# Acelogic/Retrieval-based-Voice-Conversion-MLX

Measured on AMD Instinct MI355X. Metric: audio-sec/sec (realtime factor) RVCv2 48kHz pipeline, higher is better.
Workload: dtype fp32-accurate (two-plane fp16 MFMA split); 1 GPU; C2: full RVCv2 48kHz pipeline, one 13.5 s utterance per step per GPU; samples_16k=216100, x_pad=1, f0_method=rmvpe, parallelism=dp1

## Files before the change

### retrieval-based-voice-conversion-mlx_amd/csrc/conv2d_small.hip

```cpp
#include <hip/hip_runtime.h>

#include <cstdlib>

#include "split_bf16.h"

namespace rvcx {

namespace {
typedef float f32x4 __attribute__((ext_vector_type(4)));

}

constexpr int SIT = 17;

template <int CIN, int NOUT, int PIX>
__global__ __launch_bounds__(256) void k_conv2d_small(const ConvArgs a, const int RH) {
  constexpr int CP = CIN + 4;
  constexpr int NT = NOUT / 16;
  constexpr int CG = CIN / 16;
  constexpr int TPW = PIX / 64;
  extern __shared__ __attribute__((aligned(16))) float sm[];
  const int W = a.W_out, H = a.T_out;
  const int AW = W + 2;
  float* As = sm;
// ... 396 lines not shown
                   (a.res_mode == RES_NONE || a.res_mode == RES_ADD_POST) &&
                   (a.act == ACT_NONE || a.act == ACT_RELU || a.act == ACT_LRELU) && a.w_bs == 0 && a.bias_bs == 0;
  const bool align = (a.ldx % 4 == 0) && (a.x_bs % 4 == 0) && (a.ldw % 4 == 0) && (a.w_ts % 4 == 0) &&
                     ((reinterpret_cast<uintptr_t>(a.x) & 15) == 0) && ((reinterpret_cast<uintptr_t>(a.w) & 15) == 0) &&
                     a.ldx >= a.C_in && a.ldw >= a.C_in;
  return epi && align;
}

static int s2d_nt(const ConvArgs& a) { return a.N <= 16 ? 1 : 2; }
long long small2d_wsplit_bytes(const ConvArgs& a) {
  return (long long)(a.C_in == 16 ? 5 : 9) * s2d_nt(a) * 2 * 1024 + 256;
}
hipError_t small2d_wsplit_build(const ConvArgs& a, void* out, hipStream_t s) {
  if (!conv2d_small_fits(a)) return hipErrorInvalidValue;
  hipLaunchKernelGGL(k_s2d_wsplit, dim3(1), dim3(256), 0, s, a.w, a.w_ts, a.ldw, a.N, a.C_in, s2d_nt(a),
                     static_cast<unsigned short*>(out));
  return hipGetLastError();
}

hipError_t conv2d_small(const ConvArgs& a, hipStream_t s) {
  if (a.wsplit && a.wsplit_fmt == WSPLIT_S2D) {
    hipError_t e = hipErrorInvalidValue;
    if (a.C_in == 16) e = a.N <= 16 ? launch_h16<16, 16>(a, s) : launch_h16<16, 32>(a, s);
    else e = a.N <= 16 ? launch_h16<32, 16>(a, s) : launch_h16<32, 32>(a, s);
    if (e != hipErrorInvalidValue) return e;
  }
  if (a.C_in == 16 && a.N <= 16) return launch_small<16, 16, 512>(a, s);
  if (a.C_in == 16 && a.N == 32) return launch_small<16, 32, 512>(a, s);
  if (a.C_in == 32 && a.N <= 16) return launch_small<32, 16, 256>(a, s);
  if (a.C_in == 32 && a.N == 32) return launch_small<32, 32, 256>(a, s);
  return hipErrorInvalidValue;
}

}
```

### retrieval-based-voice-conversion-mlx_amd/csrc/conv_kernels.h

```cpp
#pragma once
#include "kernel_base.h"

namespace rvcx {

enum ResMode : int {
  RES_NONE = 0,
  RES_ADD_PRE = 1,
  RES_ADD_POST = 2,
  RES_RSUB_POST = 3,
};

enum AccMode : int {
  ACC_STORE = 0,
  ACC_ADD = 1,
  ACC_ADD_DIV = 2,
};

enum OutMap : int {
  OUT_ROWS = 0,
  OUT_UPSAMPLE2D = 1,
};

enum WsplitFmt : int { WSPLIT_BF16 = 0, WSPLIT_H16 = 1, WSPLIT_S2D = 2 };

// ... 62 lines not shown
  const float* nz_w = nullptr;
  const float* nz_b = nullptr;
  int lds_pad = 0;
  const int* h_in = nullptr;
};

enum ConvKind : int { CK_WSB16 = 0, CK_WSB, CK_GS, CK_GSW, CK_RBPAIR, CK_SMALL2D, CK_EMU, CK_GEMM, CK_TINY, CK_WST,
                      CK_OTHER, CK_COUNT };
const char* conv_kind_name(int k);
enum ConvTile : int {
  TILE_NONE = -1,
  TILE_F32_128x32 = 1, TILE_F32_64x64 = 3, TILE_EMU_128x32 = 12, TILE_EMU_64x64 = 13,
  TILE_WSB_128x64 = 23, TILE_WSB_256x32 = 24, TILE_WSB_128x128 = 25, TILE_WSB_128x64_1x4 = 27, TILE_GS_64x64 = 30,
};
struct ConvForce {
  int kind = -1, tile = TILE_NONE, pipe = 0;
};
struct ConvPlan {
  ConvKind kind;
  int tile, ksplit;
  long long slab_floats;
  int wsplit_fmt;
  bool needs_image, pipe;
};
ConvPlan conv_plan(const ConvArgs& a, bool two_d, bool static_weight, const ConvForce& force = ConvForce());
hipError_t conv_run(const ConvPlan& plan, const ConvArgs& a, bool two_d, hipStream_t s, bool forced = false);
int conv_math(int requested);


bool conv2d_small_fits(const ConvArgs& a);
hipError_t conv2d_small(const ConvArgs& a, hipStream_t s);
long long small2d_wsplit_bytes(const ConvArgs& a);
hipError_t small2d_wsplit_build(const ConvArgs& a, void* out, hipStream_t s);

bool conv_wsb_eligible(const ConvArgs& a, bool two_d = false);
bool conv_wsb_tile(int cfg, int& BM, int& BN);
int conv_wsplit_npad(int N);
long long conv_wsplit_bytes(const ConvArgs& a);
hipError_t conv_wsplit_build(const ConvArgs& a, void* out, hipStream_t s);
hipError_t conv_wsb_launch(const ConvArgs& a, int cfg, hipStream_t s, bool two_d = false,
                           int ksplit = 1);

bool conv_gs_eligible(const ConvArgs& a, bool two_d);
bool conv_gs_form(const ConvArgs& a, bool two_d);
bool conv_gsw_eligible(const ConvArgs& a);
hipError_t conv_gs_launch(const ConvArgs& a, int cfg, hipStream_t s, bool two_d, int ksplit);

bool conv_wst_fits(const ConvArgs& a, bool two_d);
hipError_t conv_wst_launch(const ConvArgs& a, hipStream_t s);

struct RbPairArgs {
  const float* x = nullptr;
  long long x_bs = 0;
  const void* w1s = nullptr;
  const float* b1 = nullptr;
  const void* w2s = nullptr;
  const float* b2 = nullptr;
  int C = 0, k = 0, d = 1, T = 0, B = 1;
  float* y = nullptr;
  long long y_bs = 0;
  int acc_mode = ACC_STORE;
  float acc_div = 1.f;
  int wfmt = 0;
  int lowp = 0;
};
enum RbWfmt : int { RB_WBF16 = 0, RB_WF16 = 1 };
// ... 7 lines not shown
```

### retrieval-based-voice-conversion-mlx_amd/csrc/runtime.h

```cpp
#pragma once
#include <hip/hip_runtime.h>

#include <cstdint>
#include <cstdlib>
#include <functional>
#include <map>
#include <memory>
#include <stdexcept>
#include <string>
#include <tuple>
#include <vector>

#include "../../include/rvcx.h"
#include "rvcx_kernels.h"

namespace rvcx {

struct Error : std::runtime_error {
  int code;
  Error(int c, const std::string& m) : std::runtime_error(m), code(c) {}
};

#define RVCX_HIP(expr)                                                                                 \
  do {                                                                                                 \
// ... 342 lines not shown
                         const float* rate, const float* one_minus_rate, float* out, hipStream_t s);
void index_reconstruct_n(Ctx& c, int64_t i0, int64_t ni, float* out, hipStream_t s);
void index_build(Ctx& c, const float* x, int64_t n, int d, int64_t nlist, const rvcx_index_build_opts& o,
                 hipStream_t s);
void index_centroids(Ctx& c, float* out, hipStream_t s);
int64_t index_save(Ctx& c, void* bytes, int64_t cap);
void kmeans_assign_run(Ctx& c, const float* x, int64_t n, int d, const float* cent, int64_t nlist, int32_t* assign,
                       float* dist, hipStream_t s);
void kmeans_update_run(Ctx& c, const float* x, int64_t n, int d, const int32_t* assign, int64_t nlist, float* cent,
                       int64_t* sizes, hipStream_t s);
int64_t pipeline_forward_ex(Ctx& c, const double* audio, int64_t n, const rvcx_pipeline_opts& o,
                            const float* eps_z, const float* eps_src, uint64_t seed, float* out, int64_t cap,
                            double* f0_out, hipStream_t s, bool sizing);
int64_t pipeline_forward_batch(Ctx& c, const double* audio, int64_t n, int64_t lda, int B, const rvcx_pipeline_opts& o,
                               const int32_t* sids, const float* eps_z, const float* eps_src, uint64_t seed,
                               float* out, int64_t ldo, double* f0_out, float* hidden_out, hipStream_t s);
void pipeline_forward_rows(Ctx& c, const double* audio, const int64_t* nv, int64_t lda, int B,
                           const rvcx_pipeline_opts& o, const int32_t* sids, const float* eps_z, const float* eps_src,
                           uint64_t seed, float* out, int64_t ldo, int64_t* n_out, double* f0_out, int64_t ldf,
                           float* hidden_out, hipStream_t s, bool sizing);
int64_t pipeline_workspace_bytes(Ctx& c, int B, int64_t n, const rvcx_pipeline_opts& o, hipStream_t s);
rvcx_pipeline_opts default_pipeline_opts();
int proposed_key(const std::vector<double>& f0, double threshold);
int64_t hubert_frames(int64_t n);
void set_i32(int32_t* p, int32_t v, hipStream_t s);
void set_i32_once(Ctx& c, const std::string& name, int32_t* p, int32_t v, hipStream_t s);
hipStream_t fork_aux(Ctx& c, hipStream_t s);
bool conv_routes_wsb16(Ctx& c, const ConvArgs& a);
void join_aux(Ctx& c, hipStream_t s, hipStream_t ax);
void launch_conv(Ctx& c, const ConvArgs& a_in, bool two_d, hipStream_t s, double flops = -1.0);
ConvPlan launch_conv_test(Ctx& c, const ConvArgs& a_in, bool two_d, bool static_weight, const ConvForce& force,
                          int expect_kind, const char* who, hipStream_t s);
void launch_rb_pair(Ctx& c, const RbPairArgs& a, hipStream_t s);
inline void check(hipError_t e, const char* what) {
  if (e != hipSuccess) throw Error(RVCX_E_HIP, std::string(what) + ": " + hipGetErrorString(e));
}

}
```

### retrieval-based-voice-conversion-mlx_amd/csrc/runtime_conv.cpp

```cpp
#include <algorithm>
#include <cstdlib>
#include <cstring>
#include <string>

#include "runtime.h"

namespace rvcx {
hipStream_t Ctx::aux_stream() {
  if (!aux) {
    RVCX_HIP(hipSetDevice(device));
    RVCX_HIP(hipStreamCreateWithFlags(&aux, hipStreamNonBlocking));
    RVCX_HIP(hipEventCreateWithFlags(&ev_fork, hipEventDisableTiming));
    RVCX_HIP(hipEventCreateWithFlags(&ev_join, hipEventDisableTiming));
    RVCX_HIP(hipEventCreateWithFlags(&ev_gate, hipEventDisableTiming));
  }
  return aux;
}

unsigned* Ctx::device_status() {
  if (!status_host) {
    RVCX_HIP(hipSetDevice(device));
    void* h = nullptr;
    RVCX_HIP(hipHostMalloc(&h, 64, hipHostMallocMapped));
    std::memset(h, 0, 64);
// ... 124 lines not shown
    }
    b->bytes = bytes;
    check(rb_wsplit_build(w, C, k, b->p, s, wfmt), "rb_wsplit_build");
    RVCX_HIP(hipStreamSynchronize(s));
    slot = std::move(b);
  }
  return slot->p;
}

static hipEvent_t take_event(Ctx& c) {
  hipEvent_t e;
  if (!c.prof_pool.empty()) {
    e = c.prof_pool.back();
    c.prof_pool.pop_back();
  } else {
    RVCX_HIP(hipEventCreate(&e));
  }
  return e;
}

void launch_rb_pair(Ctx& c, const RbPairArgs& a, hipStream_t s) {
  constexpr int cfg = 0;
  if (!c.prof) {
    check(rb_pair(a, cfg, s), "rb_pair");
    return;
  }
  const double flops = 2.0 * 2.0 * a.B * (double)a.T * a.C * a.C * a.k;
  const double bytes = 4.0 * ((double)a.B * a.T * a.C * (2 + (a.acc_mode != ACC_STORE ? 1 : 0)) + 2.0 * a.k * a.C * a.C);
  Ctx::ProfRec r{take_event(c), take_event(c), flops, 0, a.T, a.C, a.C, -a.k, a.B, 1, bytes,
                 a.wfmt == RB_WF16 ? (a.lowp ? Ctx::PEAK_F16 : Ctx::PEAK_F16X2) : Ctx::PEAK_SPLIT};
  r.kind = CK_RBPAIR;
  RVCX_HIP(hipEventRecord(r.a, s));
  check(rb_pair(a, cfg, s), "rb_pair");
  RVCX_HIP(hipEventRecord(r.b, s));
  c.prof_recs.push_back(r);
}

bool conv_routes_wsb16(Ctx& c, const ConvArgs& a_in) {
  ConvArgs a = a_in;
  if (c.conv_math > 0 && a.math == 0) a.math = c.conv_math;
  const ConvPlan p = conv_plan(a, false, a.w_static || c.is_weight(a.w));
  return (p.kind == CK_WSB16 || p.kind == CK_WST) && p.wsplit_fmt == WSPLIT_H16 && p.ksplit == 1;
}

namespace {
void run_planned(Ctx& c, const ConvPlan& p, ConvArgs& a, bool two_d, bool forced, hipStream_t s, double flops) {
  if (p.ksplit > 1)
    a.ws = c.buf<float>(c.aux && s == c.aux ? "conv.splitk.aux" : "conv.splitk", (size_t)p.slab_floats, s);
  auto run = [&] {
    const hipError_t e = conv_run(p, a, two_d, s, forced);
    if (e == hipSuccess) return;
    auto n = [](long long v) { return std::to_string(v); };
    throw Error(RVCX_E_HIP, std::string(two_d ? "conv2d: " : "conv1d: ") + conv_kind_name(p.kind) + " tile " + n(p.tile) +
                                " ksplit " + n(p.ksplit) + " refused " + n(a.T_out) + " x " + n(a.W_out) + " rows, N " +
                                n(a.N) + ", C_in " + n(a.C_in) + ", " + n(a.taps) + " taps: " + hipGetErrorString(e));
  };
  if (!c.prof) return run();
  if (flops < 0) {
    const double M = two_d ? (double)a.T_out * a.W_out : (double)a.T_out;
    flops = 2.0 * M * a.N * (double)a.C_in * a.taps * a.batch * a.batch_inner;
  }
  const double in_rows = two_d ? (double)a.T_in * a.W_in : (double)a.T_in;
  const double out_el = (two_d ? (double)a.T_out * a.W_out : (double)a.T_out) * a.N * a.batch * a.batch_inner;
  const double alg_bytes = 4.0 * (in_rows * a.C_in * a.batch * a.batch_inner + (double)a.taps * a.N * a.C_in +
                                  out_el * (1 + (a.res && a.res_mode != RES_NONE ? 1 : 0) +
                                            (a.acc_mode != ACC_STORE ? 1 : 0)));
// ... 61 lines not shown
```

### retrieval-based-voice-conversion-mlx_amd/csrc/runtime_fe.cpp

```cpp
#include <cmath>
#include <utility>

#include "model_build.h"

namespace rvcx {

namespace {

constexpr int HD = 768, HHEADS = 12, HFF = 3072, HCONV = 512;
const int HK[7] = {10, 3, 3, 3, 3, 2, 2};
const int HS[7] = {5, 2, 2, 2, 2, 2, 2};
constexpr int POS_K = 128, POS_G = 16;

}

void finalize_hubert(Ctx& c) {
  const int M = 1;
  c.alloc_weight("hb.conv0", host_weight(c, M, "feature_extractor.conv_layers.0.conv.weight", {HCONV, 1, HK[0]}).v);
  for (int i = 1; i < 7; ++i)
    c.alloc_weight("hb.conv" + std::to_string(i),
                   pack_conv1d(host_weight(c, M, "feature_extractor.conv_layers." + std::to_string(i) + ".conv.weight",
                                    {HCONV, HCONV, HK[i]})));
  c.alloc_weight("hb.gn.g", host_weight(c, M, "feature_extractor.conv_layers.0.layer_norm.weight", {HCONV}).v);
  c.alloc_weight("hb.gn.b", host_weight(c, M, "feature_extractor.conv_layers.0.layer_norm.bias", {HCONV}).v);
// ... 287 lines not shown
      for (int t = 0; t < 9; ++t) v[((size_t)t * O + o) * I + i] = (float)((double)w[((size_t)o * I + i) * 9 + t] * bn.a[o]);
    bias[o] = (float)bn.b[o];
  }
  c.alloc_weight(dst + ".w", v);
  c.alloc_weight(dst + ".b", bias);
}

void block_weights(Ctx& c, const std::string& p, const std::string& q, int cin, int cout) {
  conv_bn(c, p + ".conv.0.weight", p + ".conv.1", cout, cin, q + ".c1");
  conv_bn(c, p + ".conv.3.weight", p + ".conv.4", cout, cout, q + ".c2");
  if (cin != cout) {
    c.alloc_weight(q + ".sc.w", host_weight(c, 2, p + ".shortcut.weight", {cout, cin, 1, 1}).v);
    c.alloc_weight(q + ".sc.b", host_weight(c, 2, p + ".shortcut.bias", {cout}).v);
  }
}

ConvArgs c2d(const float* x, int ldx, int H, int W, int Cin, const float* w, int N, const float* bias, float* y,
             int ldy, int B = 1, const int* hv = nullptr) {
  ConvArgs a = lin(x, ldx, H, Cin, w, N, bias, y, ldy);
  a.batch = B;
  a.h_in = hv;
  a.x_bs = (long long)H * W * ldx;
  a.y_bs = (long long)H * W * ldy;
  a.W_in = a.W_out = W;
  a.w_ts = (long long)N * Cin;
  a.taps = 9;
  a.KH = a.KW = 3;
  a.padh = a.padw = 1;
  return a;
}

void conv_block(Ctx& c, const std::string& q, const float* x, int ldx, int H, int W, int cin, int cout, float* y,
                int ldy, hipStream_t s, int B = 1, const int* hv = nullptr) {
  const size_t P = (size_t)H * W;
  float* t = c.buf<float>("rm.blk.t", (size_t)B * P * cout, s);
  ConvArgs a = c2d(x, ldx, H, W, cin, c.W(q + ".c1.w"), cout, c.W(q + ".c1.b"), t, cout, B, hv);
  a.act = ACT_RELU;
  run2(c, a, s);
  const float* res = x;
  int ldr = ldx;
  if (cin != cout) {
    float* sc = c.buf<float>("rm.blk.sc", (size_t)B * P * cout, s);
    run1(c, lin(x, ldx, (int)(B * P), cin, c.W(q + ".sc.w"), cout, c.W(q + ".sc.b"), sc, cout), s);
    res = sc;
    ldr = cout;
  }
  ConvArgs b = c2d(t, cout, H, W, cout, c.W(q + ".c2.w"), cout, c.W(q + ".c2.b"), y, ldy, B, hv);
  b.act = ACT_RELU;
  b.res = res;
  b.ldr = ldr;
  b.res_bs = (long long)P * ldr;
  b.res_mode = RES_ADD_POST;
  run2(c, b, s);
}

}

void finalize_rmvpe(Ctx& c) {
  c.alloc_weight("rm.stft", stft_weights(MEL.win));
  c.alloc_weight("rm.mel", mel_basis(MEL));
  {
    BN bn = bn_fold(c, "unet.encoder.bn", 1);
    c.host[2]["__bn0__"] = HostTensor{{(float)bn.a[0], (float)bn.b[0]}, {2}};
  }
  int cin = 1, cout = C_BASE;
  for (int i = 0; i < LEVELS; ++i) {
    for (int b = 0; b < NBLK; ++b)
      block_weights(c, "unet.encoder.layers." + std::to_string(i) + ".conv." + std::to_string(b),
                    "rm.enc" + std::to_string(i) + "." + std::to_string(b), b == 0 ? cin : cout, cout);
    cin = cout;
    cout *= 2;
  }
  const int top = C_BASE << LEVELS;
  int ci = top / 2;
  for (int i = 0; i < INTER; ++i) {
    for (int b = 0; b < NBLK; ++b)
      block_weights(c, "unet.intermediate.layers." + std::to_string(i) + ".conv." + std::to_string(b),
                    "rm.int" + std::to_string(i) + "." + std::to_string(b), b == 0 ? ci : top, top);
    ci = top;
  }
  int C = top;
  for (int i = 0; i < LEVELS; ++i) {
    const int co = C / 2;
    const std::string p = "unet.decoder.layers." + std::to_string(i);
    const std::string q = "rm.dec" + std::to_string(i);
    {
      auto& w = host_weight(c, 2, p + ".conv1.0.weight", {C, co, 3, 3}).v;
      BN bn = bn_fold(c, p + ".conv1.1", co);
// ... 306 lines not shown
```

### retrieval-based-voice-conversion-mlx_amd/rvcx/_lib.py

```python
from __future__ import annotations

import ctypes
import os
from typing import Optional

_HERE = os.path.dirname(os.path.abspath(__file__))
LIB_PATH = os.environ.get("RVCX_LIB", os.path.join(_HERE, "librvcx.so"))

RVCX_MODEL_SYNTH, RVCX_MODEL_HUBERT, RVCX_MODEL_RMVPE, RVCX_MODEL_CREPE, RVCX_MODEL_FCPE = 0, 1, 2, 3, 4

STATUS = {
    0: "RVCX_OK", -1: "RVCX_E_INVALID", -2: "RVCX_E_SHAPE", -3: "RVCX_E_HIP", -4: "RVCX_E_OOM",
    -5: "RVCX_E_STATE", -6: "RVCX_E_CAPACITY",
}


class RvcxLibraryError(ImportError):
    pass


class RvcxError(RuntimeError):
    def __init__(self, code: int, msg: str):
        super().__init__(f"{STATUS.get(code, code)}: {msg}")
        self.code = code
# ... 150 lines not shown
    "rvcx_rmvpe_batch": (i32, [vp, vp, i64, i64, i32, f32, vp, i64, P(i64), vp, vp]),
    "rvcx_rmvpe_batch_v": (i32, [vp, vp, P(i64), i64, i32, f32, vp, i64, P(i64), vp, i64, vp]),
    "rvcx_fcpe_batch_v": (i32, [vp, vp, P(i64), i64, i32, f32, i32, vp, i64, P(i64), vp, i64, vp]),
    "rvcx_rt_default_desc": (i32, [P(RtDesc)]),
    "rvcx_rt_default_opts": (i32, [P(RtOpts)]),
    "rvcx_rt_create": (i32, [vp, P(RtDesc), P(vp)]),
    "rvcx_rt_destroy": (i32, [vp, vp]),
    "rvcx_rt_geometry": (i32, [vp, P(i64)]),
    "rvcx_rt_reset": (i32, [vp, vp, vp]),
    "rvcx_rt_process": (i32, [vp, vp, vp, P(ctypes.c_int32), P(RtOpts), vp, vp, u64, vp, vp, vp, vp]),
    "rvcx_rt_process_v": (i32, [vp, vp, vp, P(ctypes.c_int32), P(RtOpts), P(ctypes.c_uint8), vp, vp, u64, vp, vp,
                                vp, vp]),
    "rvcx_rt_reset_stream": (i32, [vp, vp, i32, vp]),
    "rvcx_spectral_gate": (i32, [vp, vp, i32, i64, i64, i32, P(f32), vp, i64, vp, vp]),
    "rvcx_rt_set_clean": (i32, [vp, vp, i32, i32, f64]),
    "rvcx_device_status": (i32, [vp, vp]),
    "rvcx_index_parse": (i32, [vp, i64, P(i64), P(i64), P(i64), P(i64), ctypes.c_char_p, i64]),
    "rvcx_config_info": (i32, [vp, vp, i64, P(i64)]),
    "rvcx_profile_read_kinds": (i32, [vp, P(f64), P(f64), P(i64), P(f64), i32, P(f64), P(f64), P(f64), P(f64),
                                      P(i64)]),
    "rvcx_profile_kind_name": (ctypes.c_char_p, [i32]),
}

TEST_SIG = {
    "rvcx_set_conv_math": (i32, [vp, i32]),
    "rvcx_conv1d": (i32, [vp, vp, i64, i32, vp, vp, i32, i32, i32, i32, i32, i32, vp, i64, vp]),
    "rvcx_conv1d_gen": (i32, [vp, vp, i64, i32, vp, vp, i32, i32, i32, i32, i32, f32, i32, f32, vp, i32, f32, i32,
                              vp, vp]),
    "rvcx_conv1d_ex": (i32, [vp, P(ConvTestDesc), P(i32), P(i32), vp]),
    "rvcx_conv2d3x3": (i32, [vp, vp, i32, i32, i32, vp, vp, i32, i32, i32, vp, vp]),
    "rvcx_convtranspose2d_s2": (i32, [vp, vp, i32, i32, i32, vp, vp, i32, i32, i32, vp, vp]),
    "rvcx_conv2d3x3_v": (i32, [vp, vp, i32, P(i32), i32, i32, i32, vp, vp, i32, i32, i32, vp, vp]),
    "rvcx_convtranspose2d_s2_v": (i32, [vp, vp, i32, P(i32), i32, i32, i32, vp, vp, i32, i32, i32, vp, vp]),
    "rvcx_flash_attention": (i32, [vp, vp, i32, i32, i32, i32, f32, vp, vp, i32, vp, vp, vp]),
    "rvcx_resblock_pair": (i32, [vp, vp, i32, i64, i32, vp, vp, vp, vp, i32, i32, i32, f32, i32, vp, vp]),
    "rvcx_performer_attention": (i32, [vp, vp, vp, vp, i32, i32, vp, i32, vp, vp]),
    "rvcx_performer_attention_b": (i32, [vp, vp, vp, vp, i32, i32, i32, vp, i32, vp, vp]),
    "rvcx_performer_attention_v": (i32, [vp, vp, vp, vp, i32, i32, P(i32), i32, vp, i32, vp, vp]),
    "rvcx_fcpe_mel": (i32, [vp, vp, i64, vp, i64, P(i64), vp]),
    "rvcx_set_dec_window": (i32, [vp, i32]),
    "rvcx_dec_margin_frames": (i32, [P(SynthDesc), P(i32)]),
    "rvcx_conv_plan": (i32, [P(ConvTestDesc), P(ConvPlanForm), i32, i32, i32, i32, i32, i32, P(i32), P(i32), P(i32),
                             P(i32)]),
    "rvcx_kmeans_assign": (i32, [vp, vp, i64, i32, vp, i64, vp, vp, vp]),
    "rvcx_kmeans_update": (i32, [vp, vp, i64, i32, vp, i64, vp, vp, vp]),
    "rvcx_rt_model_rows": (i32, [vp, vp, i32, vp, i64, vp]),
    "rvcx_gru_bidir": (i32, [vp, vp, i32, i32, vp, vp, vp, vp, vp, i64, vp]),
    "rvcx_gru_bidir_v": (i32, [vp, vp, i32, P(i32), vp, vp, vp, vp, vp, i64, vp]),
    "rvcx_dec_source": (i32, [vp, i32, i32, vp, vp, u64, vp, vp]),
    "rvcx_rg_resample_dw": (i32, [vp, vp, i32, i32, i32, vp, i32, i32, vp, i32, vp]),
    "rvcx_rg_lerp_up_cat": (i32, [vp, vp, i32, i32, i32, i32, i32, f32, vp, i32, vp, i32, vp]),
    "rvcx_rg_adain": (i32, [vp, vp, i32, i32, i32, vp, vp, u64, f32, vp, i32, f32, vp]),
}

EXPORTS = list(SIG)
TEST_EXPORTS = list(TEST_SIG)

_lib: Optional[ctypes.CDLL] = None


def load(path: Optional[str] = None) -> ctypes.CDLL:
    global _lib
    if _lib is not None and path is None:
        return _lib
    p = path or LIB_PATH
    if not os.path.exists(p):
# ... 32 lines not shown
```

### retrieval-based-voice-conversion-mlx_amd/rvcx/engine_kernels.py

```python
from __future__ import annotations

import ctypes
from typing import Optional

import numpy as np

from . import _lib
from .config import SynthConfig


def _ptr(t) -> Optional[int]:
    return None if t is None else t.data_ptr()


class KernelTestMixin:
    def set_dec_window(self, on: bool):
        self._check(self.lib.rvcx_set_dec_window(self.ctx, 1 if on else 0), "set_dec_window")

    def dec_margin_frames(self, cfg: SynthConfig = None) -> int:
        d = self._synth_desc(cfg if cfg is not None else self.synth_cfg)
        m = ctypes.c_int32(0)
        rc = self.lib.rvcx_dec_margin_frames(ctypes.byref(d), ctypes.byref(m))
        if rc != 0:
            raise _lib.RvcxError(rc, "dec_margin_frames: bad synthesizer configuration")
# ... 291 lines not shown
                                                     1 if relu else 0, m, _ptr(y), self.stream()), "convtranspose2d_s2")
        return y

    def conv2d3x3_v(self, x, heights, w, bias=None, relu: bool = False, math: str = "default"):
        torch = self.torch
        x = self._dev(x, torch.float32).contiguous()
        w = torch.as_tensor(w, dtype=torch.float32)
        N, C = int(w.shape[0]), int(w.shape[1])
        wk = self._dev(w.permute(2, 3, 0, 1).reshape(9, N, C).contiguous(), torch.float32)
        b = self._dev(bias, torch.float32) if bias is not None else None
        B, H, W = (int(v) for v in x.shape[:3])
        hv = (ctypes.c_int32 * B)(*[int(v) for v in heights])
        y = torch.empty((B, H, W, N), dtype=torch.float32, device=self.device)
        m = {"default": 0, "f32": 1, "gsw": 2}[math]
        self._check(self.lib.rvcx_conv2d3x3_v(self.ctx, _ptr(x), B, hv, H, W, C, _ptr(wk), _ptr(b), N,
                                              1 if relu else 0, m, _ptr(y), self.stream()), "conv2d3x3_v")
        return y

    def convtranspose2d_s2_v(self, x, heights, w, bias=None, relu: bool = False, math: str = "default"):
        torch = self.torch
        x = self._dev(x, torch.float32).contiguous()
        wd = self._dev(torch.as_tensor(w, dtype=torch.float32).contiguous(), torch.float32)
        C, N = int(wd.shape[0]), int(wd.shape[1])
        b = self._dev(bias, torch.float32) if bias is not None else None
        B, H, W = (int(v) for v in x.shape[:3])
        hv = (ctypes.c_int32 * B)(*[int(v) for v in heights])
        y = torch.empty((B, 2 * H, 2 * W, N), dtype=torch.float32, device=self.device)
        m = {"default": 0, "f32": 1}[math]
        self._check(self.lib.rvcx_convtranspose2d_s2_v(self.ctx, _ptr(x), B, hv, H, W, C, _ptr(wd), _ptr(b), N,
                                                       1 if relu else 0, m, _ptr(y), self.stream()),
                    "convtranspose2d_s2_v")
        return y

    def flash_attention(self, qkv, n_heads: int, qscale: float, rel_k=None, rel_v=None, window: int = 0, mask=None):
        torch = self.torch
        q = self._dev(qkv, torch.float32)
        B, T, H3 = (int(v) for v in q.shape)
        dk = H3 // 3 // n_heads
        rk = None if rel_k is None else self._dev(rel_k, torch.float32)
        rv = None if rel_v is None else self._dev(rel_v, torch.float32)
        mk = None if mask is None else self._dev(mask, torch.float32)
        y = torch.empty((B, T, H3 // 3), dtype=torch.float32, device=self.device)
        self._check(self.lib.rvcx_flash_attention(self.ctx, _ptr(q), B, T, int(n_heads), dk, float(qscale), _ptr(rk),
                                                  _ptr(rv), int(window), _ptr(mk), _ptr(y), self.stream()),
                    "flash_attention")
        return y

    def resblock_pair(self, x, w1, b1, w2, b2, dilation: int, acc=None, acc_mode: int = 0, acc_div: float = 1.0,
                      cfg: int = 0):
        torch = self.torch
        x = self._dev(x, torch.float32)
        B, T, C = (int(v) for v in x.shape)
        k = int(np.shape(w1)[2])
        w1k = self._dev(torch.as_tensor(w1, dtype=torch.float32).permute(2, 0, 1).contiguous(), torch.float32)
        w2k = self._dev(torch.as_tensor(w2, dtype=torch.float32).permute(2, 0, 1).contiguous(), torch.float32)
        b1d, b2d = self._dev(b1, torch.float32), self._dev(b2, torch.float32)
        y = (self._dev(acc, torch.float32).clone() if acc is not None
             else torch.empty((B, T, C), dtype=torch.float32, device=self.device))
        self._check(self.lib.rvcx_resblock_pair(self.ctx, _ptr(x), B, T, C, _ptr(w1k), _ptr(b1d), _ptr(w2k), _ptr(b2d),
                                                k, dilation, acc_mode, float(acc_div), cfg, _ptr(y), self.stream()),
                    "resblock_pair")
        return y
```

Measured before the change: 1155 audio-sec/sec.

## Fuse RMVPE U-Net residual conv block into one kernel with LDS-resident intermediate

Adds a fused HIP kernel that runs both 3x3 convolutions of a U-Net residual block in one launch. The first conv's ReLU output stays in LDS as a split fp16 tile with a halo, so the intermediate tensor never goes through global memory, and bias, ReLU and the residual add are applied in the epilogue. The aim is to cut one launch and the write and re-read of the intermediate activation. In exchange it recomputes the halo, uses a large LDS footprint that can lower occupancy, and is on by default behind RVCX_UNET_FUSE, falling back to the two separate convs when the shape does not fit.

```diff
diff --git a/retrieval-based-voice-conversion-mlx_amd/csrc/conv2d_small.hip b/retrieval-based-voice-conversion-mlx_amd/csrc/conv2d_small.hip
--- a/retrieval-based-voice-conversion-mlx_amd/csrc/conv2d_small.hip
+++ b/retrieval-based-voice-conversion-mlx_amd/csrc/conv2d_small.hip
@@ -452,4 +452,312 @@
   return hipErrorInvalidValue;
 }
 
-}
+namespace {
+typedef unsigned u32x4 __attribute__((ext_vector_type(4)));
+constexpr int UB_TW = 16;
+constexpr int UB_NTHR = 256;
+constexpr int ub_th(int cin, int n) { return cin == 16 && n == 16 ? 16 : 8; }
+
+constexpr size_t ub_wbytes(int nbv1, int nbv2, int nthr) {
+  const int r2 = (nbv2 + nthr - 1) / nthr * nthr;
+  return (size_t)(nbv1 > r2 ? nbv1 : r2) * 16;
+}
+
+__device__ __forceinline__ int ub_rows_in(const UnetBlockArgs& a, int b) {
+  typedef const int __attribute__((address_space(4))) * const_ip;
+  return a.h_in ? ((const_ip)a.h_in)[b] : a.H;
+}
+
+template <int C, int NT, int PS>
+__device__ __forceinline__ void ub_mma(const char* As, const char* Bs, const int AW, const int zoff,
+                                       const int (&pbase)[2], const int lane, f32x4 (&acc)[2][NT],
+                                       f32x4 (&acc2)[2][NT]) {
+  constexpr int KS = C == 16 ? 5 : 9;
+  const int g = lane >> 4;
+#pragma unroll
+  for (int ks = 0; ks < KS; ++ks) {
+    const int tap = C == 16 ? 2 * ks + (g >> 1) : ks;
+    const int toff = ((tap / 3) * AW + tap % 3) * PS;
+    f16x8 bh[NT], bl[NT];
+#pragma unroll
+    for (int t = 0; t < NT; ++t) {
+      const char* src = Bs + ((size_t)((ks * NT + t) * 2) * 64 + lane) * 16;
+      bh[t] = *reinterpret_cast<const f16x8*>(src);
+      bl[t] = *reinterpret_cast<const f16x8*>(src + 64 * 16);
+    }
+#pragma unroll
+    for (int p = 0; p < 2; ++p) {
+      const int ao = (C == 16 && tap >= 9) ? zoff : pbase[p] + toff;
+      const f16x8 ah = *reinterpret_cast<const f16x8*>(As + ao);
+      const f16x8 al = *reinterpret_cast<const f16x8*>(As + ao + C * 2);
+#pragma unroll
+      for (int t = 0; t < NT; ++t) {
+        acc[p][t] = __builtin_amdgcn_mfma_f32_16x16x32_f16(ah, bh[t], acc[p][t], 0, 0, 0);
+        f32x4 c = acc2[p][t];
+        c = __builtin_amdgcn_mfma_f32_16x16x32_f16(al, bh[t], c, 0, 0, 0);
+        c = __builtin_amdgcn_mfma_f32_16x16x32_f16(ah, bl[t], c, 0, 0, 0);
+        acc2[p][t] = c;
+      }
+    }
+  }
+}
+}
+
+template <int CIN, int N>
+__global__ __launch_bounds__(UB_NTHR) void k_unet_block(const UnetBlockArgs a) {
+  constexpr int NTHR = UB_NTHR;
+  constexpr int TH = ub_th(CIN, N), TW = UB_TW;
+  constexpr int KS1 = CIN == 16 ? 5 : 9, KS2 = N == 16 ? 5 : 9;
+  constexpr int NT = N / 16;
+  constexpr int PS1 = CIN * 4 + 16, PS2 = N * 4 + 16;
+  constexpr int XW = TW + 4, XPIX = (TH + 4) * XW;
+  constexpr int TWD = TW + 2, TPIX = (TH + 2) * TWD;
+  constexpr int NWAVE = NTHR / 64;
+  constexpr int NBV1 = KS1 * NT * 2 * 64, NBV2 = KS2 * NT * 2 * 64;
+  constexpr int BIT1 = (NBV1 + NTHR - 1) / NTHR, BIT2 = (NBV2 + NTHR - 1) / NTHR;
+  constexpr int XIT = (XPIX * (CIN / 4) + NTHR - 1) / NTHR;
+  constexpr int F1P = ((TPIX + 15) / 16 + 1) / 2;
+  constexpr int P1 = (F1P + NWAVE - 1) / NWAVE;
+  constexpr int P2 = TH / 2 / NWAVE;
+  static_assert(TW == 16 && (TH / 2) % NWAVE == 0, "a conv2 fragment is one tile row, a wave takes whole pairs");
+  extern __shared__ __attribute__((aligned(16))) char smh[];
+  constexpr int XB = (XPIX + 1) * PS1, TB = (TPIX + 1) * PS2;
+  char* Xs = smh;
+  char* Ts = smh;
+  char* Bs = smh + (XB > TB ? XB : TB);
+  const int W = a.W, H = a.H;
+  const int b = blockIdx.z;
+  const int Hi = ub_rows_in(a, b);
+  const int h0 = blockIdx.y * TH, w0 = blockIdx.x * TW;
+  const float* X = a.x + (long long)b * a.x_bs;
+  const int tid = threadIdx.x, lane = tid & 63, wave = tid >> 6;
+  const int li = lane & 15, g = lane >> 4;
+
+  const float* R = a.res + (long long)b * a.res_bs;
+  f32x4 rv[P2][2][NT];
+#pragma unroll
+  for (int ps = 0; ps < P2; ++ps)
+#pragma unroll
+    for (int p = 0; p < 2; ++p) {
+      const int gh = h0 + 2 * (ps * NWAVE + wave) + p;
+#pragma unroll
+      for (int t = 0; t < NT; ++t)
+#pragma unroll
+        for (int i = 0; i < 4; ++i)
+          rv[ps][p][t][i] = R[((long long)(gh < H ? gh : 0) * W + (w0 + 4 * g + i)) * a.ldr + t * 16 + li];
+    }
+  const float* inv1 = static_cast<const float*>(a.w1s) + NBV1 * 4;
+  const float* inv2 = static_cast<const float*>(a.w2s) + NBV2 * 4;
+  float inv1v[NT], inv2v[NT], b1v[NT], b2v[NT];
+#pragma unroll
+  for (int t = 0; t < NT; ++t) {
+    inv1v[t] = inv1[t * 16 + li];
+    inv2v[t] = inv2[t * 16 + li];
+    b1v[t] = a.b1[t * 16 + li];
+    b2v[t] = a.b2[t * 16 + li];
+  }
+  u32x4 w2v[BIT2];
+  {
+    f32x4 v[XIT];
+#pragma unroll
+    for (int it = 0; it < XIT; ++it) {
+      const int idx = it * NTHR + tid;
+      const int q = idx % (CIN / 4);
+      const int pix = idx / (CIN / 4);
+      const int r = pix / XW, cc = pix - r * XW;
+      const int gh = h0 - 2 + r, gw = w0 - 2 + cc;
+      const bool ok = idx < XPIX * (CIN / 4) && gh >= 0 && gh < Hi && gw >= 0 && gw < W;
+      v[it] = *reinterpret_cast<const f32x4*>(X + ((long long)(ok ? gh : 0) * W + (ok ? gw : 0)) * a.ldx + 4 * q);
+      if (!ok) v[it] = f32x4{0.f, 0.f, 0.f, 0.f};
+    }
+    uint4 bv[BIT1];
+    const uint4* wimg1 = static_cast<const uint4*>(a.w1s);
+    const u32x4* wimg2 = static_cast<const u32x4*>(a.w2s);
+#pragma unroll
+    for (int it = 0; it < BIT1; ++it) {
+      const int idx = it * NTHR + tid;
+      bv[it] = wimg1[idx < NBV1 ? idx : 0];
+    }
+#pragma unroll
+    for (int it = 0; it < BIT2; ++it) {
+      const int idx = it * NTHR + tid;
+      w2v[it] = wimg2[idx < NBV2 ? idx : 0];
+    }
+#pragma unroll
+    for (int it = 0; it < BIT1; ++it) {
+      const int idx = it * NTHR + tid;
+      if (idx < NBV1) reinterpret_cast<uint4*>(Bs)[idx] = bv[it];
+    }
+#pragma unroll
+    for (int it = 0; it < XIT; ++it) {
+      const int idx = it * NTHR + tid;
+      if (idx < XPIX * (CIN / 4)) {
+        f32x4 val = v[it];
+#pragma unroll
+        for (int j = 0; j < 4; ++j) val[j] *= H16_XS;
+        char* row = Xs + (size_t)(idx / (CIN / 4)) * PS1;
+        const int c4 = 4 * (idx % (CIN / 4));
+        uint2 hh, ll;
+        hh.x = pk_f16(val[0], val[1]);
+        hh.y = pk_f16(val[2], val[3]);
+        ll.x = pk_f16((val[0] - f16lo_f(hh.x)) * H16_LO, (val[1] - f16hi_f(hh.x)) * H16_LO);
+        ll.y = pk_f16((val[2] - f16lo_f(hh.y)) * H16_LO, (val[3] - f16hi_f(hh.y)) * H16_LO);
+        *reinterpret_cast<uint2*>(row + c4 * 2) = hh;
+        *reinterpret_cast<uint2*>(row + CIN * 2 + c4 * 2) = ll;
+      }
+    }
+    if (tid < PS1 / 16) reinterpret_cast<uint4*>(Xs + (size_t)XPIX * PS1)[tid] = make_uint4(0u, 0u, 0u, 0u);
+  }
+  __syncthreads();
+
+  f32x4 tv[P1][2][NT];
+#pragma unroll
+  for (int ps = 0; ps < P1; ++ps) {
+    const int q0 = 2 * (ps * NWAVE + wave) * 16;
+    if (q0 >= TPIX) continue;
+    f32x4 acc[2][NT], acc2[2][NT];
+    int pbase[2];
+#pragma unroll
+    for (int p = 0; p < 2; ++p) {
+#pragma unroll
+      for (int t = 0; t < NT; ++t) acc[p][t] = acc2[p][t] = f32x4{0.f, 0.f, 0.f, 0.f};
+      const int q = q0 + p * 16 + li;
+      const int qc = q < TPIX ? q : TPIX - 1;
+      pbase[p] = ((qc / TWD) * XW + qc % TWD) * PS1 + (CIN == 16 ? 16 * (g & 1) : 16 * g);
+    }
+    ub_mma<CIN, NT, PS1>(Xs, Bs, XW, XPIX * PS1, pbase, lane, acc, acc2);
+#pragma unroll
+    for (int t = 0; t < NT; ++t) {
+      const float bn = b1v[t];
+      const float inv = inv1v[t];
+#pragma unroll
+      for (int p = 0; p < 2; ++p) {
+        f32x4 v;
+#pragma unroll
+        for (int i = 0; i < 4; ++i) v[i] = (acc[p][t][i] + acc2[p][t][i] * H16_LO_INV) * inv;
+#pragma unroll
+        for (int i = 0; i < 4; ++i) v[i] += bn;
+#pragma unroll
+        for (int i = 0; i < 4; ++i) v[i] = v[i] > 0.f ? v[i] : 0.f;
+#pragma unroll
+        for (int i = 0; i < 4; ++i) {
+          const int q = q0 + p * 16 + 4 * g + i;
+          const int r = q / TWD, cc = q - r * TWD;
+          const int gh = h0 - 1 + r, gw = w0 - 1 + cc;
+          const bool in = gh >= 0 && gh < Hi && gw >= 0 && gw < W;
+          tv[ps][p][t][i] = in ? v[i] : 0.f;
+        }
+      }
+    }
+  }
+  __syncthreads();
+#pragma unroll
+  for (int ps = 0; ps < P1; ++ps) {
+    const int q0 = 2 * (ps * NWAVE + wave) * 16;
+    if (q0 >= TPIX) continue;
+#pragma unroll
+    for (int t = 0; t < NT; ++t) {
+      const int n = t * 16 + li;
+#pragma unroll
+      for (int p = 0; p < 2; ++p)
+#pragma unroll
+        for (int i = 0; i < 4; ++i) {
+          const int q = q0 + p * 16 + 4 * g + i;
+          const float val = tv[ps][p][t][i] * H16_XS;
+          const unsigned hh = pk_f16(val, 0.f);
+          const unsigned ll = pk_f16((val - f16lo_f(hh)) * H16_LO, 0.f);
+          if (q < TPIX) {
+            char* row = Ts + (size_t)q * PS2;
+            *reinterpret_cast<unsigned short*>(row + 2 * n) = (unsigned short)hh;
+            *reinterpret_cast<unsigned short*>(row + N * 2 + 2 * n) = (unsigned short)ll;
+          }
+        }
+    }
+  }
+  if (tid < PS2 / 16) reinterpret_cast<uint4*>(Ts + (size_t)TPIX * PS2)[tid] = make_uint4(0u, 0u, 0u, 0u);
+#pragma unroll
+  for (int it = 0; it < BIT2; ++it) {
+    const int idx = it * NTHR + tid;
+    reinterpret_cast<u32x4*>(Bs)[idx] = w2v[it];
+  }
+  __syncthreads();
+
+  float* Y = a.y + (long long)b * a.y_bs;
+#pragma unroll
+  for (int ps = 0; ps < P2; ++ps) {
+    const int f0 = 2 * (ps * NWAVE + wave);
+    f32x4 acc[2][NT], acc2[2][NT];
+    int pbase[2];
+#pragma unroll
+    for (int p = 0; p < 2; ++p) {
+#pragma unroll
+      for (int t = 0; t < NT; ++t) acc[p][t] = acc2[p][t] = f32x4{0.f, 0.f, 0.f, 0.f};
+      pbase[p] = ((f0 + p) * TWD + li) * PS2 + (N == 16 ? 16 * (g & 1) : 16 * g);
+    }
+    ub_mma<N, NT, PS2>(Ts, Bs, TWD, TPIX * PS2, pbase, lane, acc, acc2);
+#pragma unroll
+    for (int t = 0; t < NT; ++t) {
+      const int n = t * 16 + li;
+      const float bn = b2v[t];
+      const float inv = inv2v[t];
+#pragma unroll
+      for (int p = 0; p < 2; ++p) {
+        const int gh = h0 + f0 + p;
+        f32x4 v;
+#pragma unroll
+        for (int i = 0; i < 4; ++i) v[i] = (acc[p][t][i] + acc2[p][t][i] * H16_LO_INV) * inv;
+#pragma unroll
+        for (int i = 0; i < 4; ++i) v[i] += bn;
+#pragma unroll
+        for (int i = 0; i < 4; ++i) v[i] = v[i] > 0.f ? v[i] : 0.f;
+#pragma unroll
+        for (int i = 0; i < 4; ++i) v[i] = v[i] + rv[ps][p][t][i];
+        if (gh < H) {
+#pragma unroll
+          for (int i = 0; i < 4; ++i) Y[((long long)gh * W + (w0 + 4 * g + i)) * a.ldy + n] = v[i];
+        }
+      }
+    }
+  }
+}
+
+namespace {
+template <int CIN, int N>
+hipError_t launch_unet_block(const UnetBlockArgs& a, hipStream_t s) {
+  constexpr int NTHR = UB_NTHR, TH = ub_th(CIN, N);
+  constexpr int KS1 = CIN == 16 ? 5 : 9, KS2 = N == 16 ? 5 : 9;
+  constexpr size_t xb = (size_t)((TH + 4) * (UB_TW + 4) + 1) * (CIN * 4 + 16);
+  constexpr size_t tb = (size_t)((TH + 2) * (UB_TW + 2) + 1) * (N * 4 + 16);
+  constexpr size_t lds = (xb > tb ? xb : tb) + ub_wbytes(KS1 * (N / 16) * 2 * 64, KS2 * (N / 16) * 2 * 64, NTHR);
+  static_assert(lds <= 160 * 1024, "LDS per workgroup");
+  auto kern = k_unet_block<CIN, N>;
+  static bool lds_set = false;
+  if (!lds_set) {
+    hipError_t e = hipFuncSetAttribute(reinterpret_cast<const void*>(kern),
+                                       hipFuncAttributeMaxDynamicSharedMemorySize, (int)lds);
+    if (e != hipSuccess) return e;
+    lds_set = true;
+  }
+  dim3 grid(a.W / UB_TW, (a.H + TH - 1) / TH, a.batch);
+  hipLaunchKernelGGL(kern, grid, dim3(NTHR), lds, s, a);
+  return hipGetLastError();
+}
+}
+
+bool unet_block_fits(const UnetBlockArgs& a) {
+  const bool shape = (a.C_in == 16 || a.C_in == 32) && (a.N == 16 || a.N == 32) && a.H >= 1 && a.W >= UB_TW &&
+                     a.W % UB_TW == 0 && a.batch >= 1 && a.batch <= 65535 && (a.H + 7) / 8 <= 65535;
+  const bool ptrs = a.x && a.y && a.res && a.w1s && a.w2s && a.b1 && a.b2 && a.y != a.x && a.y != a.res;
+  const bool align = a.ldx % 4 == 0 && a.x_bs % 4 == 0 && a.ldx >= a.C_in && a.ldr >= a.N && a.ldy >= a.N &&
+                     (reinterpret_cast<uintptr_t>(a.x) & 15) == 0 && (reinterpret_cast<uintptr_t>(a.w1s) & 15) == 0 &&
+                     (reinterpret_cast<uintptr_t>(a.w2s) & 15) == 0;
+  return shape && ptrs && align;
+}
+
+hipError_t unet_block(const UnetBlockArgs& a, hipStream_t s) {
+  if (!unet_block_fits(a)) return hipErrorInvalidValue;
+  if (a.C_in == 16) return a.N == 16 ? launch_unet_block<16, 16>(a, s) : launch_unet_block<16, 32>(a, s);
+  return a.N == 16 ? launch_unet_block<32, 16>(a, s) : launch_unet_block<32, 32>(a, s);
+}
+
+}
diff --git a/retrieval-based-voice-conversion-mlx_amd/csrc/conv_kernels.h b/retrieval-based-voice-conversion-mlx_amd/csrc/conv_kernels.h
--- a/retrieval-based-voice-conversion-mlx_amd/csrc/conv_kernels.h
+++ b/retrieval-based-voice-conversion-mlx_amd/csrc/conv_kernels.h
@@ -118,6 +118,23 @@
 hipError_t conv2d_small(const ConvArgs& a, hipStream_t s);
 long long small2d_wsplit_bytes(const ConvArgs& a);
 hipError_t small2d_wsplit_build(const ConvArgs& a, void* out, hipStream_t s);
+struct UnetBlockArgs {
+  const float* x = nullptr;
+  long long x_bs = 0;
+  int ldx = 0;
+  const void *w1s = nullptr, *w2s = nullptr;
+  const float *b1 = nullptr, *b2 = nullptr;
+  const float* res = nullptr;
+  long long res_bs = 0;
+  int ldr = 0;
+  float* y = nullptr;
+  long long y_bs = 0;
+  int ldy = 0;
+  int H = 0, W = 0, C_in = 0, N = 0, batch = 1;
+  const int* h_in = nullptr;
+};
+bool unet_block_fits(const UnetBlockArgs& a);
+hipError_t unet_block(const UnetBlockArgs& a, hipStream_t s);
 
 bool conv_wsb_eligible(const ConvArgs& a, bool two_d = false);
 bool conv_wsb_tile(int cfg, int& BM, int& BN);
diff --git a/retrieval-based-voice-conversion-mlx_amd/csrc/runtime.h b/retrieval-based-voice-conversion-mlx_amd/csrc/runtime.h
--- a/retrieval-based-voice-conversion-mlx_amd/csrc/runtime.h
+++ b/retrieval-based-voice-conversion-mlx_amd/csrc/runtime.h
@@ -398,6 +398,13 @@
 ConvPlan launch_conv_test(Ctx& c, const ConvArgs& a_in, bool two_d, bool static_weight, const ConvForce& force,
                           int expect_kind, const char* who, hipStream_t s);
 void launch_rb_pair(Ctx& c, const RbPairArgs& a, hipStream_t s);
+void launch_unet_block(Ctx& c, const UnetBlockArgs& a, hipStream_t s);
+struct UnetBlockW {
+  const float *w1, *b1, *w2, *b2, *scw, *scb;
+};
+void unet_conv_block(Ctx& c, const UnetBlockW& w, const float* x, int ldx, int H, int W, int cin, int cout, float* y,
+                     int ldy, hipStream_t s, int B, const int* hv, bool fuse, bool test);
+bool unet_fuse_default();
 inline void check(hipError_t e, const char* what) {
   if (e != hipSuccess) throw Error(RVCX_E_HIP, std::string(what) + ": " + hipGetErrorString(e));
 }
diff --git a/retrieval-based-voice-conversion-mlx_amd/csrc/runtime_conv.cpp b/retrieval-based-voice-conversion-mlx_amd/csrc/runtime_conv.cpp
--- a/retrieval-based-voice-conversion-mlx_amd/csrc/runtime_conv.cpp
+++ b/retrieval-based-voice-conversion-mlx_amd/csrc/runtime_conv.cpp
@@ -180,6 +180,22 @@
   r.kind = CK_RBPAIR;
   RVCX_HIP(hipEventRecord(r.a, s));
   check(rb_pair(a, cfg, s), "rb_pair");
+  RVCX_HIP(hipEventRecord(r.b, s));
+  c.prof_recs.push_back(r);
+}
+
+void launch_unet_block(Ctx& c, const UnetBlockArgs& a, hipStream_t s) {
+  if (!c.prof) {
+    check(unet_block(a, s), "unet_block");
+    return;
+  }
+  const double M = (double)a.H * a.W;
+  const double flops = 2.0 * M * a.N * (double)(a.C_in + a.N) * 9 * a.batch;
+  const double bytes = 4.0 * (M * a.batch * (a.C_in + 2.0 * a.N) + 9.0 * a.N * (a.C_in + a.N));
+  Ctx::ProfRec r{take_event(c), take_event(c), flops, 1, a.H * a.W, a.N, a.C_in, 9, a.batch, 1, bytes, Ctx::PEAK_F16X2};
+  r.kind = CK_SMALL2D;
+  RVCX_HIP(hipEventRecord(r.a, s));
+  check(unet_block(a, s), "unet_block");
   RVCX_HIP(hipEventRecord(r.b, s));
   c.prof_recs.push_back(r);
 }
diff --git a/retrieval-based-voice-conversion-mlx_amd/csrc/runtime_fe.cpp b/retrieval-based-voice-conversion-mlx_amd/csrc/runtime_fe.cpp
--- a/retrieval-based-voice-conversion-mlx_amd/csrc/runtime_fe.cpp
+++ b/retrieval-based-voice-conversion-mlx_amd/csrc/runtime_fe.cpp
@@ -343,28 +343,99 @@
 
 void conv_block(Ctx& c, const std::string& q, const float* x, int ldx, int H, int W, int cin, int cout, float* y,
                 int ldy, hipStream_t s, int B = 1, const int* hv = nullptr) {
+  const bool sc = cin != cout;
+  const UnetBlockW w{c.W(q + ".c1.w"), c.W(q + ".c1.b"), c.W(q + ".c2.w"), c.W(q + ".c2.b"),
+                     sc ? c.W(q + ".sc.w") : nullptr, sc ? c.W(q + ".sc.b") : nullptr};
+  unet_conv_block(c, w, x, ldx, H, W, cin, cout, y, ldy, s, B, hv, unet_fuse_default(), false);
+}
+
+}
+
+bool unet_fuse_default() {
+  const char* e = rvcx_knob("RVCX_UNET_FUSE");
+  return e ? std::atoi(e) != 0 : true;
+}
+
+void unet_conv_block(Ctx& c, const UnetBlockW& w, const float* x, int ldx, int H, int W, int cin, int cout, float* y,
+                     int ldy, hipStream_t s, int B, const int* hv, bool fuse, bool test) {
+  const char* who = "rvcx_unet_block";
   const size_t P = (size_t)H * W;
   float* t = c.buf<float>("rm.blk.t", (size_t)B * P * cout, s);
-  ConvArgs a = c2d(x, ldx, H, W, cin, c.W(q + ".c1.w"), cout, c.W(q + ".c1.b"), t, cout, B, hv);
+  ConvArgs a = c2d(x, ldx, H, W, cin, w.w1, cout, w.b1, t, cout, B, hv);
   a.act = ACT_RELU;
-  run2(c, a, s);
   const float* res = x;
   int ldr = ldx;
-  if (cin != cout) {
-    float* sc = c.buf<float>("rm.blk.sc", (size_t)B * P * cout, s);
-    run1(c, lin(x, ldx, (int)(B * P), cin, c.W(q + ".sc.w"), cout, c.W(q + ".sc.b"), sc, cout), s);
-    res = sc;
+  float* scb = w.scw ? c.buf<float>("rm.blk.sc", (size_t)B * P * cout, s) : nullptr;
+  if (scb) {
+    res = scb;
     ldr = cout;
   }
-  ConvArgs b = c2d(t, cout, H, W, cout, c.W(q + ".c2.w"), cout, c.W(q + ".c2.b"), y, ldy, B, hv);
+  ConvArgs b = c2d(t, cout, H, W, cout, w.w2, cout, w.b2, y, ldy, B, hv);
   b.act = ACT_RELU;
   b.res = res;
   b.ldr = ldr;
   b.res_bs = (long long)P * ldr;
   b.res_mode = RES_ADD_POST;
+  auto shortcut = [&] {
+    if (scb) run1(c, lin(x, ldx, (int)(B * P), cin, w.scw, cout, w.scb, scb, cout), s);
+  };
+  bool fused = false;
+  if (fuse && w.b1 && w.b2) {
+    ConvArgs a1 = a, b1 = b;
+    if (c.conv_math > 0) a1.math = b1.math = c.conv_math;
+    const ConvPlan pa = conv_plan(a1, true, test || c.is_weight(a1.w));
+    const ConvPlan pb = conv_plan(b1, true, test || c.is_weight(b1.w));
+    auto s2d = [&](const ConvPlan& p) {
+      return p.kind == CK_SMALL2D && p.wsplit_fmt == WSPLIT_S2D && (test || p.needs_image);
+    };
+    UnetBlockArgs u;
+    u.x = x;
+    u.x_bs = a.x_bs;
+    u.ldx = ldx;
+    u.b1 = w.b1;
+    u.b2 = w.b2;
+    u.res = res;
+    u.res_bs = b.res_bs;
+    u.ldr = ldr;
+    u.y = y;
+    u.y_bs = b.y_bs;
+    u.ldy = ldy;
+    u.H = H;
+    u.W = W;
+    u.C_in = cin;
+    u.N = cout;
+    u.batch = B;
+    u.h_in = hv;
+    u.w1s = u.w2s = x;
+    if (s2d(pa) && s2d(pb) && unet_block_fits(u)) {
+      a1.wsplit_fmt = b1.wsplit_fmt = WSPLIT_S2D;
+      if (test) {
+        void* i1 = c.buf<char>("conv.test.blk.w1s", (size_t)conv_wsplit_bytes(a1), s);
+        void* i2 = c.buf<char>("conv.test.blk.w2s", (size_t)conv_wsplit_bytes(b1), s);
+        check(conv_wsplit_build(a1, i1, s), "conv_wsplit_build");
+        check(conv_wsplit_build(b1, i2, s), "conv_wsplit_build");
+        u.w1s = i1;
+        u.w2s = i2;
+      } else {
+        u.w1s = c.wsplit_for(a1, s);
+        u.w2s = c.wsplit_for(b1, s);
+      }
+      shortcut();
+      launch_unet_block(c, u, s);
+      fused = true;
+    }
+  }
+  if (fused) return;
+  if (test && fuse) throw Error(RVCX_E_SHAPE, std::string(who) + ": the fused kernel does not admit this block");
+  if (test) {
+    launch_conv_test(c, a, true, true, ConvForce(), CK_SMALL2D, who, s);
+    shortcut();
+    launch_conv_test(c, b, true, true, ConvForce(), CK_SMALL2D, who, s);
+    return;
+  }
+  run2(c, a, s);
+  shortcut();
   run2(c, b, s);
-}
-
 }
 
 void finalize_rmvpe(Ctx& c) {
diff --git a/retrieval-based-voice-conversion-mlx_amd/rvcx/_lib.py b/retrieval-based-voice-conversion-mlx_amd/rvcx/_lib.py
--- a/retrieval-based-voice-conversion-mlx_amd/rvcx/_lib.py
+++ b/retrieval-based-voice-conversion-mlx_amd/rvcx/_lib.py
@@ -206,6 +206,7 @@
     "rvcx_convtranspose2d_s2": (i32, [vp, vp, i32, i32, i32, vp, vp, i32, i32, i32, vp, vp]),
     "rvcx_conv2d3x3_v": (i32, [vp, vp, i32, P(i32), i32, i32, i32, vp, vp, i32, i32, i32, vp, vp]),
     "rvcx_convtranspose2d_s2_v": (i32, [vp, vp, i32, P(i32), i32, i32, i32, vp, vp, i32, i32, i32, vp, vp]),
+    "rvcx_unet_block": (i32, [vp, vp, i32, P(i32), i32, i32, i32, vp, vp, vp, vp, vp, vp, i32, i32, vp, vp]),
     "rvcx_flash_attention": (i32, [vp, vp, i32, i32, i32, i32, f32, vp, vp, i32, vp, vp, vp]),
     "rvcx_resblock_pair": (i32, [vp, vp, i32, i64, i32, vp, vp, vp, vp, i32, i32, i32, f32, i32, vp, vp]),
     "rvcx_performer_attention": (i32, [vp, vp, vp, vp, i32, i32, vp, i32, vp, vp]),
diff --git a/retrieval-based-voice-conversion-mlx_amd/rvcx/engine_kernels.py b/retrieval-based-voice-conversion-mlx_amd/rvcx/engine_kernels.py
--- a/retrieval-based-voice-conversion-mlx_amd/rvcx/engine_kernels.py
+++ b/retrieval-based-voice-conversion-mlx_amd/rvcx/engine_kernels.py
@@ -347,6 +347,29 @@
                     "convtranspose2d_s2_v")
         return y
 
+    def unet_block(self, x, w1, b1, w2, b2, wsc=None, bsc=None, heights=None, fused: bool = True):
+        torch = self.torch
+        x = self._dev(x, torch.float32).contiguous()
+        B, H, W, C = (int(v) for v in x.shape)
+        N = int(np.shape(w1)[0])
+
+        def taps(w):
+            w = torch.as_tensor(w, dtype=torch.float32)
+            return self._dev(w.permute(2, 3, 0, 1).reshape(9, int(w.shape[0]), int(w.shape[1])).contiguous(),
+                             torch.float32)
+
+        w1k, w2k = taps(w1), taps(w2)
+        b1d, b2d = self._dev(b1, torch.float32), self._dev(b2, torch.float32)
+        wscd = None if wsc is None else self._dev(torch.as_tensor(wsc, dtype=torch.float32).reshape(N, C).contiguous(),
+                                                  torch.float32)
+        bscd = None if bsc is None else self._dev(bsc, torch.float32)
+        hv = None if heights is None else (ctypes.c_int32 * B)(*[int(v) for v in heights])
+        y = torch.empty((B, H, W, N), dtype=torch.float32, device=self.device)
+        self._check(self.lib.rvcx_unet_block(self.ctx, _ptr(x), B, hv, H, W, C, _ptr(w1k), _ptr(b1d), _ptr(w2k),
+                                             _ptr(b2d), _ptr(wscd), _ptr(bscd), N, 1 if fused else 0, _ptr(y),
+                                             self.stream()), "unet_block")
+        return y
+
     def flash_attention(self, qkv, n_heads: int, qscale: float, rel_k=None, rel_v=None, window: int = 0, mask=None):
         torch = self.torch
         q = self._dev(qkv, torch.float32)
```

Measured after the change: 1175 audio-sec/sec, median of 6. 1.02x the previous value.
